# NeptuneHub/AudioMuse-AI

Measured on NVIDIA H100. Metric: tracks_per_sec_analysed_10s_48khz, higher is better.
Workload: dtype bf16

## Files before the change

### audiomuse-ai_b200/csrc/debug/block_debug.cu

```cuda
#include "../common.cuh"
#include "../depthwise.cuh"
#include "../fused_block.cuh"
#include "../gemm_wgmma.cuh"
#include "../model_spec.cuh"
#include "../../../include/audiomuse_b200_debug.h"

#include <vector>

namespace {

template <typename T>
int upload(am::DevBuf<T>& d, const void* h, size_t n) {
  AM_TRY(d.alloc(n));
  AM_CUDA(cudaMemcpy(d.p, h, n * sizeof(T), cudaMemcpyHostToDevice));
  return AM_OK;
}

template <typename T>
int download(void* h, const am::DevBuf<T>& d, size_t n) {
  AM_CUDA(cudaMemcpy(h, d.p, n * sizeof(T), cudaMemcpyDeviceToHost));
  return AM_OK;
}

}

extern "C" AM_API int am_debug_block(int path, int B, int H, int W, int cin_p, int cmid_p, int cout_p, int stride,
                                     int has_expand, int residual, const uint16_t* X, const uint16_t* W1,
                                     const float* b1, const float* wd, const float* bd, const uint16_t* W2,
                                     const float* b2, uint16_t* Y, uint16_t* E_out, uint16_t* D_out, int* info) {
  using namespace am;
  AM_CHECK(path >= 0 && path <= 2, "am_debug_block: path %d", path);
  AM_CHECK(B > 0 && H > 0 && W > 0 && (stride == 1 || stride == 2), "am_debug_block: bad shape");
  AM_CHECK(cin_p > 0 && cmid_p > 0 && cout_p > 0 && cin_p % 16 == 0 && cmid_p % 16 == 0 && cout_p % 16 == 0,
           "am_debug_block: channel counts must be positive multiples of 16");
  AM_CHECK(has_expand || cin_p == cmid_p, "am_debug_block: a block without expansion has cin_p == cmid_p");
  AM_CHECK(!residual || (stride == 1 && cin_p == cout_p), "am_debug_block: a residual needs stride 1, cin_p == cout_p");
  AM_CHECK(info, "am_debug_block: NULL info");

  fused::Plan pl;
  fused::BlockDesc d{};
  if (path != 1) {
    d.H = H;
    d.W = W;
    d.cin_p = cin_p;
    d.cmid_p = cmid_p;
    d.cout_p = cout_p;
    d.stride = stride;
    d.has_expand = has_expand ? 1 : 0;
    d.residual = residual ? 1 : 0;
    AM_CHECK(fused::plan(d, &pl), "am_debug_block: the fused kernel does not take this block");
    if (path == 2) {
      *info = pl.tile_h;
      return AM_OK;
    }
  }

  AM_CHECK(X && wd && bd && W2 && b2 && Y && (!has_expand || (W1 && b1)), "am_debug_block: NULL operand");
  AM_TRY(ensure_init());
  const int Ho = (H - 1) / stride + 1, Wo = (W - 1) / stride + 1;
  const size_t n_x = (size_t)B * H * W * cin_p, n_e = (size_t)B * H * W * cmid_p;
  const size_t n_d = (size_t)B * Ho * Wo * cmid_p, n_y = (size_t)B * Ho * Wo * cout_p;
  const std::vector<float> h_wd(wd, wd + (size_t)9 * cmid_p), h_bd(bd, bd + cmid_p);

  DevBuf<__nv_bfloat16> dX, dW1, dW2, dE, dD, dY;
  DevBuf<float> db1, dwd, dbd, db2, dparams;
  AM_TRY(upload(dX, X, n_x));
  AM_TRY(upload(dW2, W2, (size_t)cout_p * cmid_p));
  AM_TRY(upload(db2, b2, cout_p));
  if (has_expand) {
    AM_TRY(upload(dW1, W1, (size_t)cmid_p * cin_p));
    AM_TRY(upload(db1, b1, cmid_p));
  }
  AM_TRY(dY.alloc(n_y));
  AM_CUDA(cudaMemset(dY.p, 0xff, n_y * 2));

  if (path == 0) {
    const std::vector<float> h_b1 = has_expand ? std::vector<float>(b1, b1 + cmid_p) : std::vector<float>();
    const std::vector<float> packed = fused::pack_params(h_wd, h_bd, has_expand ? &h_b1 : nullptr, cmid_p);
    AM_TRY(upload(dparams, packed.data(), packed.size()));
    AM_TRY(fused::run(d, pl, dX.p, has_expand ? dW1.p : nullptr, dparams.p, dW2.p, db2.p, dY.p, B, nullptr));
    *info = pl.stages;
  } else {
    AM_TRY(upload(dwd, wd, (size_t)9 * cmid_p));
    AM_TRY(upload(dbd, bd, cmid_p));
    AM_TRY(dD.alloc(n_d));
    AM_CUDA(cudaMemset(dD.p, 0xff, n_d * 2));
    const __nv_bfloat16* dw_in = dX.p;
    if (has_expand) {
      AM_TRY(dE.alloc(n_e));
      AM_CUDA(cudaMemset(dE.p, 0xff, n_e * 2));
      gemm::Epilogue ep;
      ep.bias = db1.p;
      ep.act = kActRelu6;
      AM_TRY(gemm::gemm_bf16(dX.p, (int64_t)B * H * W, cin_p, dW1.p, cmid_p, cin_p, cin_p, dE.p, cmid_p, false, ep,
                             false, nullptr));
      dw_in = dE.p;
    }
    const bool fp16 = dw3x3_fp16_safe(h_wd, h_bd, cmid_p, has_expand != 0);
    AM_TRY(dw3x3(dw_in, B, H, W, cmid_p, stride, dwd.p, dbd.p, fp16, dD.p, nullptr, info));
    gemm::Epilogue ep;
    ep.bias = db2.p;
    if (residual) {
      ep.residual = dX.p;
      ep.ld_res = cout_p;
    }
    AM_TRY(gemm::gemm_bf16(dD.p, (int64_t)B * Ho * Wo, cmid_p, dW2.p, cout_p, cmid_p, cmid_p, dY.p, cout_p, false, ep,
                           false, nullptr));
  }
  AM_CUDA(cudaDeviceSynchronize());
  AM_TRY(download(Y, dY, n_y));
  if (path == 1 && E_out && has_expand) AM_TRY(download(E_out, dE, n_e));
  if (path == 1 && D_out) AM_TRY(download(D_out, dD, n_d));
  return AM_OK;
}
```

### audiomuse-ai_b200/csrc/fused_block.cu

```cuda
#include "fused_block.cuh"

#include <type_traits>

#include "gemm_wgmma.cuh"
#include "tma_pipeline.cuh"

namespace am {
namespace fused {

using namespace ptx;

constexpr int kTile = 8;
constexpr int kTallTile = 16;
constexpr int kChunk = 64;
constexpr int kMaxCout = 256;
constexpr int kMaxStages = 4;
constexpr size_t kSmemMax = 232448;
constexpr uint32_t kConsumerBar = 1;
constexpr int kParamRows = 9 + 1 + 1;
constexpr uint32_t kDwBytes = kParamRows * kChunk * 4;
using Ring = pipe::Ring<kMaxStages>;

__host__ __device__ constexpr int halo(int S) { return (kTile - 1) * S + 3; }
__host__ __device__ constexpr int halo_h(int S, int th) { return (th - 1) * S + 3; }
__host__ __device__ constexpr int halo_px(int S, int th) { return halo_h(S, th) * halo(S); }
__host__ __device__ constexpr int halo_rows(int S, int th) {
  return th == kTile ? (halo_px(S, th) + 63) / 64 * 64 : (halo_px(S, th) + 7) / 8 * 8;
}
__host__ __device__ constexpr int en0(int px) { return ((px + 7) / 8 + 1) / 2 * 8; }
__host__ __device__ constexpr int en1(int px) { return (px + 7) / 8 * 8 - en0(px); }

constexpr uint32_t round1k(uint32_t v) { return (v + 1023u) & ~1023u; }

__device__ __forceinline__ int e_off(int p, int g) { return p * 64 + ((g ^ (p & 7)) << 3); }

__device__ __forceinline__ uint32_t sw128(uint32_t row, uint32_t chunk) {
  return (row << 7) + (((chunk ^ row) & 7u) << 4);
}

struct Layout {
  uint32_t stage, w2, dw;
  uint32_t xs, a2, e, bars, extra;
  int hr;
  int th;
  int stages;
  size_t smem;
};

static Layout layout(int S, int th, bool has_expand, int cin_p, int cout_p, int stages) {
  const uint32_t hr = (uint32_t)halo_rows(S, th), hpx = (uint32_t)halo_px(S, th);
  const uint32_t kbx = has_expand ? (uint32_t)((cin_p + 63) / 64) : 0u;
  const uint32_t n2 = (uint32_t)((cout_p + 63) / 64 * 64);
  Layout l;
  l.w2 = has_expand ? kbx * kChunk * 128 : round1k(hpx * 128);
  l.dw = l.w2 + n2 * 128;
  l.stage = round1k(l.dw + kDwBytes);
  l.xs = 0;
  l.a2 = l.xs + kbx * hr * 128;
  l.e = l.a2 + (uint32_t)(th * kTile * 128);
  l.bars = l.e + (has_expand ? hpx * 128 : 0u);
  l.extra = l.bars + 2 * sizeof(uint64_t);
  l.hr = (int)hr;
  l.th = th;
  l.stages = stages;
  l.smem = Ring::smem_bytes(l.stage, stages, l.extra);
  return l;
}

struct Args {
  const __nv_bfloat16* X;
  const float* params;
  const float* b2;
  __nv_bfloat16* Y;
  int H, W, Ho, Wo, tiles_y, tiles_x, num_tiles;
  int cin_p, cmid_p, cout_p, residual;
  Layout l;
};

enum Phase { kRingWait, kHaloWait, kExpandMma, kExpandEpi, kDepthwise, kProjectMma, kBarrier, kEpilogue, kIssue, kNumPhases };
#ifdef AM_FUSED_PHASES
static const char* const kPhaseNames[kNumPhases] = {"ring_wait", "halo_wait", "expand_mma", "expand_epi", "depthwise",
                                                     "project_mma", "barrier", "epilogue", "issue"};
__device__ unsigned long long g_phase_cycles[3][kNumPhases];
__device__ __forceinline__ long long clock_now() {
  long long v;
  asm volatile("mov.u64 %0, %%clock64;" : "=l"(v));
  return v;
}
struct PhaseClock {
  uint32_t acc[kNumPhases];
  long long t;
  __device__ __forceinline__ PhaseClock() : acc{}, t(clock_now()) {}
  __device__ __forceinline__ void lap(Phase p) {
    const long long n = clock_now();
    acc[p] += (uint32_t)(n - t);
    t = n;
  }
  __device__ __forceinline__ void flush(int wg) {
    for (int p = 0; p < kNumPhases; ++p) atomicAdd(&g_phase_cycles[wg][p], (unsigned long long)acc[p]);
  }
};
#else
struct PhaseClock {
  __device__ __forceinline__ void lap(Phase) {}
  __device__ __forceinline__ void flush(int) {}
};
#endif

template <int S, bool kExpand>
__global__ void __launch_bounds__(pipe::kThreads, 1)
fused_block_kernel(const __grid_constant__ CUtensorMap map_x, const __grid_constant__ CUtensorMap map_w1,
                   const __grid_constant__ CUtensorMap map_w2, const Args a) {
  extern __shared__ __align__(1024) uint8_t smem_raw[];
  constexpr int HALO = halo(S);
  constexpr int PX8 = halo_px(S, kTile), PXT = halo_px(S, kTallTile);
  const bool tall = S == 1 && a.l.th == kTallTile;
  const int hpx = tall ? PXT : PX8, hr = a.l.hr;
  Ring ring(smem_raw, a.l.stage, a.l.stages, a.l.extra);
  uint8_t* own = ring.extra();
  uint8_t* xs = own + a.l.xs;
  uint8_t* a2 = own + a.l.a2;
  uint64_t* xs_full = reinterpret_cast<uint64_t*>(own + a.l.bars);
  uint64_t* xs_empty = xs_full + 1;

  const int per_img = a.tiles_y * a.tiles_x;
  const int kbx = (a.cin_p + 63) / 64;
  const int n2_blocks = (a.cout_p + 63) / 64;

  if (threadIdx.x == 0) {
    prefetch_tensormap(&map_x);
    if (kExpand) prefetch_tensormap(&map_w1);
    prefetch_tensormap(&map_w2);
    mbar_init(xs_full, 1);
    mbar_init(xs_empty, pipe::kConsumerThreads);
    ring.init();
  }
  __syncthreads();

  if (threadIdx.x < 128) {
    regs_producer();
    if (threadIdx.x < 32 && elect_one_sync()) {
      PhaseClock clk;
      uint32_t xs_phase = 0;
      for (int tile = blockIdx.x; tile < a.num_tiles; tile += gridDim.x) {
        const int b = tile / per_img, ty = (tile % per_img) / a.tiles_x, tx = tile % a.tiles_x;
        const int gy0 = ty * a.l.th * S - 1, gx0 = tx * kTile * S - 1;
        if (kExpand) {
          clk.lap(kIssue);
          mbar_wait(xs_empty, xs_phase ^ 1);
          clk.lap(kHaloWait);
          mbar_expect_tx(xs_full, (uint32_t)(kbx * hpx * 128));
          for (int kb = 0; kb < kbx; ++kb) tma_load_4d(xs + kb * hr * 128, &map_x, xs_full, kb * 64, gx0, gy0, b);
          xs_phase ^= 1;
        }
        for (int c0 = 0; c0 < a.cmid_p; c0 += kChunk) {
          const uint32_t tx_bytes = (kExpand ? (uint32_t)kbx * kChunk * 128 : (uint32_t)hpx * 128) +
                                    (uint32_t)n2_blocks * 64 * 128 + kDwBytes;
          clk.lap(kIssue);
          const Ring::Slot s = ring.acquire(tx_bytes);
          clk.lap(kRingWait);
          if (kExpand) {
            for (int kb = 0; kb < kbx; ++kb) tma_load_2d(s.smem + kb * kChunk * 128, &map_w1, s.bar, kb * 64, c0);
          } else {
            tma_load_4d(s.smem, &map_x, s.bar, c0, gx0, gy0, b);
          }
          tma_load_2d(s.smem + a.l.w2, &map_w2, s.bar, c0, 0);
          bulk_load(s.smem + a.l.dw, a.params + (int64_t)c0 * kParamRows, kDwBytes, s.bar);
        }
      }
      clk.lap(kIssue);
      clk.flush(0);
    }
    return;
  }
  regs_consumer();
  const int ct = threadIdx.x - 128;
  const int wg = __shfl_sync(0xffffffffu, ct >> 7, 0), wt = ct & 127;
  const int warp = wt >> 5, lane = wt & 31, quad = lane & 3;
  __nv_bfloat16* e_own = reinterpret_cast<__nv_bfloat16*>(own + a.l.e);
  const int nchunks = (a.cmid_p + kChunk - 1) / kChunk;
  const bool ahead = a.l.stages > 1;

  auto with_tile = [&](auto f) {
    if constexpr (S == 1) {
      if (tall) return f(std::integral_constant<int, kTallTile>{});
    }
    return f(std::integral_constant<int, kTile>{});
  };

  const int half = a.cout_p / 2;
  const int proj_n = tall ? a.cout_p : half;
  const int proj_col = tall ? 0 : wg * half;
  const int proj_row = tall ? 64 * wg : 0;

  constexpr int kAcc1 = en0(S == 1 ? PXT : PX8) / 2;
  float acc1[kAcc1];
  float acc2[kMaxCout / 4];
#pragma unroll
  for (int i = 0; i < kAcc1; ++i) acc1[i] = 0.f;
#pragma unroll
  for (int i = 0; i < kMaxCout / 4; ++i) acc2[i] = 0.f;

  auto expand_issue = [&](const uint8_t* stage) {
    const uint32_t w1 = smem_u32(stage);
    auto issue = [&](auto width, int p0) {
      const uint32_t px = smem_u32(xs) + (uint32_t)(p0 * 128);
      for (int kb = 0; kb < kbx; ++kb) {
        const uint64_t da = make_smem_desc(w1 + (uint32_t)(kb * kChunk * 128));
        const uint64_t db = make_smem_desc(px + (uint32_t)(kb * hr * 128));
        const int ksteps = min(4, (a.cin_p - kb * 64) / 16);
        for (int ks = 0; ks < ksteps; ++ks)
          wgmma_into<decltype(width)::value>(acc1, da + (uint64_t)(ks * 2), db + (uint64_t)(ks * 2),
                                             (kb | ks) ? 1u : 0u);
      }
    };
    wgmma_fence();
    with_tile([&](auto th) {
      constexpr int PX = halo_px(S, decltype(th)::value);
      if (wg == 0) issue(std::integral_constant<int, en0(PX)>{}, 0);
      else issue(std::integral_constant<int, en1(PX)>{}, en0(PX));
    });
    wgmma_commit();
  };
  auto inside_mask = [&](int gy0, int gx0) {
    return with_tile([&](auto th) {
      constexpr int EN0 = en0(halo_px(S, decltype(th)::value));
      int p0 = wg * EN0 + 2 * quad;
      asm volatile("" : "+r"(p0));
      uint64_t m = 0;
#pragma unroll
      for (int j = 0; j < EN0 / 8; ++j)
#pragma unroll
        for (int k = 0; k < 2; ++k) {
          const int p = p0 + 8 * j + k;
          const int gy = gy0 + p / HALO, gx = gx0 + p % HALO;
          if (gy >= 0 && gy < a.H && gx >= 0 && gx < a.W) m |= 1ull << (2 * j + k);
        }
      return m;
    });
  };
  auto expand_epilogue = [&](const uint8_t* stage, int nch, uint64_t inside) {
    reg_fence(acc1);
    const float* b1 = reinterpret_cast<const float*>(stage + a.l.dw) + 10 * kChunk;
    const int r = 16 * warp + (lane >> 2);
    const float bias[2] = {b1[r], b1[r + 8]};
    const uint32_t keep[2] = {r < nch ? ~0u : 0u, r + 8 < nch ? ~0u : 0u};
    auto pack = [&](int j, int h) {
      const uint32_t bits = (uint32_t)(inside >> (2 * j));
      const uint32_t mask = ((bits & 1u) * 0xffffu | (bits & 2u) * 0x7fff8000u) & keep[h];
      const __nv_bfloat162 v = __floats2bfloat162_rn(relu6f(acc1[4 * j + 2 * h] + bias[h]),
                                                     relu6f(acc1[4 * j + 2 * h + 1] + bias[h]));
      return *reinterpret_cast<const uint32_t*>(&v) & mask;
    };
    auto store = [&](auto wgc, auto th) {
      constexpr int HPX = halo_px(S, decltype(th)::value);
      constexpr int P0 = decltype(wgc)::value * en0(HPX);
      constexpr int NG = (decltype(wgc)::value ? en1(HPX) : en0(HPX)) / 8;
      constexpr int NFULL = (HPX - P0) / 8 < NG ? (HPX - P0) / 8 : NG;
      const int mi = lane >> 3;
      const uint32_t e_base = smem_u32(e_own);
#pragma unroll
      for (int j = 0; j + 1 < NFULL; j += 2) {
        const int p = P0 + 8 * (j + (mi >> 1)) + (lane & 7);
        stmatrix_x4_trans(e_base + 2 * e_off(p, 2 * warp + (mi & 1)), pack(j, 0), pack(j, 1), pack(j + 1, 0),
                          pack(j + 1, 1));
      }
      if (NFULL % 2) {
        const int p = P0 + 8 * (NFULL - 1) + (lane & 7);
        stmatrix_x2_trans(e_base + 2 * e_off(p, 2 * warp + (mi & 1)), pack(NFULL - 1, 0), pack(NFULL - 1, 1));
      }
#pragma unroll
      for (int j = NFULL; j < NG; ++j)
#pragma unroll
        for (int h = 0; h < 2; ++h) {
          const uint32_t v = pack(j, h);
#pragma unroll
          for (int k = 0; k < 2; ++k) {
            const int p = P0 + 8 * j + 2 * quad + k;
            if (p < HPX)
              reinterpret_cast<uint16_t*>(e_own)[e_off(p, 2 * warp + h) + (lane >> 2)] = (uint16_t)(v >> (16 * k));
          }
        }
    };
    with_tile([&](auto th) {
      if (wg == 0) store(std::integral_constant<int, 0>{}, th);
      else store(std::integral_constant<int, 1>{}, th);
    });
  };

  PhaseClock clk;
  uint32_t xs_phase = 0;
  for (int tile = blockIdx.x; tile < a.num_tiles; tile += gridDim.x) {
    const int b = tile / per_img, ty = (tile % per_img) / a.tiles_x, tx = tile % a.tiles_x;
    const int oy0 = ty * a.l.th, ox0 = tx * kTile;
    const int gy0 = oy0 * S - 1, gx0 = ox0 * S - 1;
    const uint64_t inside = kExpand ? inside_mask(gy0, gx0) : 0;
    if (kExpand) {
      mbar_wait(xs_full, xs_phase);
      xs_phase ^= 1;
      clk.lap(kHaloWait);
      const uint8_t* s0 = ring.wait_ptr();
      clk.lap(kRingWait);
      expand_issue(s0);
      wgmma_wait<0>();
      clk.lap(kExpandMma);
      expand_epilogue(s0, min(kChunk, a.cmid_p), inside);
      if (nchunks == 1) mbar_arrive(xs_empty);
      clk.lap(kExpandEpi);
    }

    for (int c = 0; c < nchunks; ++c) {
      const int c0 = c * kChunk, nch = min(kChunk, a.cmid_p - c0);
      const bool next = kExpand && c + 1 < nchunks;
      uint8_t* sp = ring.wait_ptr();
      clk.lap(kRingWait);
      const float* dwp = reinterpret_cast<const float*>(sp + a.l.dw);
      const __nv_bfloat16* e = kExpand ? e_own : reinterpret_cast<const __nv_bfloat16*>(sp);
      named_bar_sync(kConsumerBar, pipe::kConsumerThreads);
      clk.lap(kBarrier);
      const uint8_t* sn = nullptr;
      if (next && ahead) {
        sn = ring.wait_ahead_ptr();
        clk.lap(kRingWait);
        expand_issue(sn);
        clk.lap(kExpandMma);
      }

      with_tile([&](auto th) {
        constexpr int TH = decltype(th)::value, HH = halo_h(S, TH);
        const int ox = ct >> 5, cp = lane, g = cp >> 2;
        uint8_t* arow = a2 + sw128(ox, g) + 4 * (cp & 3);
        auto put = [&](int oy, uint32_t v) { *reinterpret_cast<uint32_t*>(arow + oy * kTile * 128) = v; };
        if (2 * cp < nch) {
          float2 w[9];
#pragma unroll
          for (int t = 0; t < 9; ++t) w[t] = *reinterpret_cast<const float2*>(dwp + t * kChunk + 2 * cp);
          const float2 bias = *reinterpret_cast<const float2*>(dwp + 9 * kChunk + 2 * cp);
          float2 acc[TH];
#pragma unroll
          for (int oy = 0; oy < TH; ++oy) acc[oy] = bias;
          auto out = [&](int oy) {
            const __nv_bfloat162 o = __floats2bfloat162_rn(relu6f(acc[oy].x), relu6f(acc[oy].y));
            return *reinterpret_cast<const uint32_t*>(&o);
          };
          const __nv_bfloat16* col[8];
#pragma unroll
          for (int k = 0; k < 8; ++k) col[k] = e + ox * S * 64 + ((g ^ ((ox * S + k) & 7)) << 3) + 2 * (cp & 3);
#pragma unroll
          for (int iy = 0; iy < HH; ++iy) {
            float2 v[3];
#pragma unroll
            for (int dx = 0; dx < 3; ++dx) {
              const int d = iy * HALO + dx;
              v[dx] = __bfloat1622float2(*reinterpret_cast<const __nv_bfloat162*>(col[d & 7] + d * 64));
            }
#pragma unroll
            for (int dy = 0; dy < 3; ++dy) {
              if (iy < dy || (iy - dy) % S != 0 || (iy - dy) / S >= TH) continue;
              const int oy = (iy - dy) / S;
#pragma unroll
              for (int dx = 0; dx < 3; ++dx) {
                acc[oy].x = fmaf(v[dx].x, w[dy * 3 + dx].x, acc[oy].x);
                acc[oy].y = fmaf(v[dx].y, w[dy * 3 + dx].y, acc[oy].y);
              }
            }
            if constexpr (TH != kTile) {
              if (iy >= 2) put(iy - 2, out(iy - 2));
            }
          }
          if constexpr (TH == kTile) {
#pragma unroll
            for (int oy = 0; oy < TH; ++oy) put(oy, out(oy));
          }
        } else {
#pragma unroll
          for (int oy = 0; oy < TH; ++oy) put(oy, 0u);
        }
      });
      fence_proxy_async();
      clk.lap(kDepthwise);
      named_bar_sync(kConsumerBar, pipe::kConsumerThreads);
      clk.lap(kBarrier);

      wgmma_fence();
      {
        const uint64_t da = make_smem_desc(smem_u32(a2) + (uint32_t)(proj_row * 128));
        const uint64_t db = make_smem_desc(smem_u32(sp) + a.l.w2 + (uint32_t)(proj_col * 128));
        auto project = [&](auto width) {
          for (int ks = 0; ks < nch / 16; ++ks)
            wgmma_into<decltype(width)::value>(acc2, da + (uint64_t)(ks * 2), db + (uint64_t)(ks * 2),
                                               (c0 | ks) ? 1u : 0u);
        };
        switch (proj_n) {
          case 8: project(std::integral_constant<int, 8>{}); break;
          case 16: project(std::integral_constant<int, 16>{}); break;
          case 24: project(std::integral_constant<int, 24>{}); break;
          case 32: project(std::integral_constant<int, 32>{}); break;
          case 40: project(std::integral_constant<int, 40>{}); break;
          case 48: project(std::integral_constant<int, 48>{}); break;
          case 56: project(std::integral_constant<int, 56>{}); break;
          case 64: project(std::integral_constant<int, 64>{}); break;
          case 72: project(std::integral_constant<int, 72>{}); break;
          case 80: project(std::integral_constant<int, 80>{}); break;
          case 88: project(std::integral_constant<int, 88>{}); break;
          case 96: project(std::integral_constant<int, 96>{}); break;
          case 104: project(std::integral_constant<int, 104>{}); break;
          case 112: project(std::integral_constant<int, 112>{}); break;
          case 120: project(std::integral_constant<int, 120>{}); break;
          case 128: project(std::integral_constant<int, 128>{}); break;
        }
      }
      wgmma_commit();
      clk.lap(kProjectMma);

      if (next && !ahead) {
        wgmma_wait<0>();
        ring.release();
        sn = ring.wait_ptr();
        clk.lap(kRingWait);
        expand_issue(sn);
      }
      wgmma_wait<0>();
      reg_fence(acc2);
      if (!next || ahead) ring.release();
      clk.lap(kProjectMma);
      if (next) {
        expand_epilogue(sn, min(kChunk, a.cmid_p - c0 - kChunk), inside);
        if (c + 2 == nchunks) mbar_arrive(xs_empty);
        clk.lap(kExpandEpi);
      }
    }

    {
      constexpr int J = kMaxCout / 16;
      bool in[2];
      int64_t pix[2];
#pragma unroll
      for (int h = 0; h < 2; ++h) {
        const int px = proj_row + warp * 16 + (lane >> 2) + 8 * h;
        const int oy = oy0 + (px >> 3), ox = ox0 + (px & 7);
        in[h] = oy < a.Ho && ox < a.Wo;
        pix[h] = ((int64_t)b * a.Ho + oy) * a.Wo + ox;
      }
      float2 bias[J];
      uint32_t res[2][J];
#pragma unroll
      for (int j = 0; j < J; ++j) {
        bias[j] = make_float2(0.f, 0.f);
        res[0][j] = res[1][j] = 0u;
        if (8 * j >= proj_n) continue;
        const int n = proj_col + 8 * j + 2 * quad;
        bias[j] = make_float2(__ldg(&a.b2[n]), __ldg(&a.b2[n + 1]));
#pragma unroll
        for (int h = 0; h < 2; ++h)
          if (a.residual && in[h]) res[h][j] = *reinterpret_cast<const uint32_t*>(a.X + pix[h] * a.cin_p + n);
      }
#pragma unroll
      for (int h = 0; h < 2; ++h) {
        if (!in[h]) continue;
#pragma unroll
        for (int j = 0; j < J; ++j) {
          if (8 * j >= proj_n) break;
          const int n = proj_col + 8 * j + 2 * quad;
          float f0 = acc2[4 * j + 2 * h] + bias[j].x;
          float f1 = acc2[4 * j + 2 * h + 1] + bias[j].y;
          if (a.residual) {
            f0 += __uint_as_float(res[h][j] << 16);
            f1 += __uint_as_float(res[h][j] & 0xffff0000u);
          }
          *reinterpret_cast<__nv_bfloat162*>(a.Y + pix[h] * a.cout_p + n) = __floats2bfloat162_rn(f0, f1);
        }
      }
    }
    clk.lap(kEpilogue);
  }
  if (wt == 0) clk.flush(1 + wg);
}

static bool fits(const BlockDesc& d) {
  const size_t hr = (size_t)halo_rows(d.stride, kTile);
  const size_t kbx = d.has_expand ? (size_t)((d.cin_p + 63) / 64) : 0;
  const size_t n2 = (size_t)((d.cout_p + 63) / 64 * 64);
  const size_t set = kbx * hr * 128 + kbx * kChunk * 128 + n2 * 128 + 64 * 128 + hr * 128;
  return set + 1024 <= kSmemMax;
}

bool plan(const BlockDesc& d, Plan* out) {
  if (d.stride != 1 && d.stride != 2) return false;
  if (d.cout_p > kMaxCout || d.cout_p % 16 || d.cmid_p % 16 || d.cin_p % 16) return false;
  if (!d.has_expand && d.cin_p != d.cmid_p) return false;
  if (d.residual && (d.stride != 1 || d.cin_p != d.cout_p)) return false;
  if (!fits(d)) return false;
  auto deepest = [&](int th) {
    Layout l = layout(d.stride, th, d.has_expand != 0, d.cin_p, d.cout_p, kMaxStages);
    for (int s = kMaxStages - 1; s >= 1 && l.smem > kSmemMax; --s)
      l = layout(d.stride, th, d.has_expand != 0, d.cin_p, d.cout_p, s);
    return l;
  };
  Layout l = deepest(kTile);
  if (d.stride == 1 && d.cout_p <= 128) {
    const Layout t = deepest(kTallTile);
    if (t.smem <= kSmemMax && t.stages == l.stages) l = t;
  }
  out->stages = l.stages;
  out->tile_h = l.th;
  out->smem_bytes = l.smem;
  return out->smem_bytes <= kSmemMax;
}

template <int S, bool kExpand>
static int launch(const CUtensorMap& mx, const CUtensorMap& m1, const CUtensorMap& m2, const Args& a, size_t smem,
                  cudaStream_t st) {
  AM_TRY((allow_dynamic_smem<fused_block_kernel<S, kExpand>>(kSmemMax)));
  const int grid = std::max(1, std::min(a.num_tiles, sm_count()));
#ifdef AM_FUSED_PHASES
  void* counters = nullptr;
  AM_CUDA(cudaGetSymbolAddress(&counters, g_phase_cycles));
  AM_CUDA(cudaMemsetAsync(counters, 0, sizeof(g_phase_cycles), st));
#endif
  AM_LAUNCH((fused_block_kernel<S, kExpand>), grid, pipe::kThreads, smem, st, mx, m1, m2, a);
#ifdef AM_FUSED_PHASES
  unsigned long long c[3][kNumPhases];
  AM_CUDA(cudaStreamSynchronize(st));
  AM_CUDA(cudaMemcpyFromSymbol(c, g_phase_cycles, sizeof(c)));
  std::fprintf(stderr, "fused_phases H=%d W=%d cin=%d cmid=%d cout=%d S=%d stages=%d grid=%d tiles=%d", a.H, a.W,
               a.cin_p, a.cmid_p, a.cout_p, S, a.l.stages, grid, a.num_tiles);
  for (int w = 0; w < 3; ++w)
    for (int p = 0; p < kNumPhases; ++p) std::fprintf(stderr, " wg%d.%s=%llu", w, kPhaseNames[p], c[w][p]);
  std::fprintf(stderr, "\n");
#endif
  return AM_OK;
}

std::vector<float> pack_params(const std::vector<float>& wd, const std::vector<float>& bd, const std::vector<float>* b1,
                               int c_p) {
  const int chunks = (c_p + kChunk - 1) / kChunk;
  std::vector<float> out((size_t)chunks * kParamRows * kChunk, 0.f);
  for (int c = 0; c < c_p; ++c) {
    float* q = &out[((size_t)(c / kChunk) * kParamRows) * kChunk + c % kChunk];
    for (int t = 0; t < 9; ++t) q[t * kChunk] = wd[(size_t)t * c_p + c];
    q[9 * kChunk] = bd[c];
    if (b1) q[10 * kChunk] = (*b1)[c];
  }
  return out;
}

int run(const BlockDesc& d, const Plan& p, const __nv_bfloat16* X, const __nv_bfloat16* W1, const float* params,
        const __nv_bfloat16* W2, const float* b2, __nv_bfloat16* Y, int B, cudaStream_t st) {
  AM_CHECK(X && params && W2 && b2 && Y && (!d.has_expand || W1), "fused block: NULL operand");
  auto aligned16 = [](const void* q) { return (reinterpret_cast<uintptr_t>(q) & 15) == 0; };
  AM_CHECK(aligned16(X) && aligned16(W2) && aligned16(params) && (!d.has_expand || aligned16(W1)),
           "fused block: operands must be 16-byte aligned (TMA)");
  Args a{};
  a.X = X;
  a.params = params;
  a.b2 = b2;
  a.Y = Y;
  a.H = d.H;
  a.W = d.W;
  a.Ho = (d.H - 1) / d.stride + 1;
  a.Wo = (d.W - 1) / d.stride + 1;
  AM_CHECK(p.tile_h == kTile || (p.tile_h == kTallTile && d.stride == 1 && d.cout_p <= 128),
           "fused block: plan does not match the block");
  a.tiles_y = (a.Ho + p.tile_h - 1) / p.tile_h;
  a.tiles_x = (a.Wo + kTile - 1) / kTile;
  const int64_t tiles = (int64_t)B * a.tiles_y * a.tiles_x;
  AM_CHECK(tiles < ((int64_t)1 << 31), "fused block: %lld tiles is too many for one launch", (long long)tiles);
  a.num_tiles = (int)tiles;
  a.cin_p = d.cin_p;
  a.cmid_p = d.cmid_p;
  a.cout_p = d.cout_p;
  a.residual = d.residual;
  const Layout l = layout(d.stride, p.tile_h, d.has_expand != 0, d.cin_p, d.cout_p, p.stages);
  AM_CHECK(l.smem == p.smem_bytes, "fused block: plan does not match the block");
  a.l = l;

  CUtensorMap mx, m1, m2;
  AM_TRY(gemm::encode_map_nhwc_bf16(&mx, X, B, d.H, d.W, d.cin_p, halo(d.stride), halo_h(d.stride, p.tile_h), true));
  AM_TRY(gemm::encode_map_bf16(&m2, W2, d.cmid_p, d.cout_p, d.cmid_p, (d.cout_p + 63) / 64 * 64));
  if (d.has_expand) AM_TRY(gemm::encode_map_bf16(&m1, W1, d.cin_p, d.cmid_p, d.cin_p, kChunk));
  else m1 = m2;
  if (d.stride == 1) return d.has_expand ? launch<1, true>(mx, m1, m2, a, l.smem, st) : launch<1, false>(mx, m1, m2, a, l.smem, st);
  return d.has_expand ? launch<2, true>(mx, m1, m2, a, l.smem, st) : launch<2, false>(mx, m1, m2, a, l.smem, st);
}

}
}
```

Baseline: 12090.

## Split depthwise rows across lanes for narrow chunks and stage output through smem

```diff
diff --git a/audiomuse-ai_b200/csrc/debug/block_debug.cu b/audiomuse-ai_b200/csrc/debug/block_debug.cu
--- a/audiomuse-ai_b200/csrc/debug/block_debug.cu
+++ b/audiomuse-ai_b200/csrc/debug/block_debug.cu
@@ -29,7 +29,7 @@
                                      const float* b1, const float* wd, const float* bd, const uint16_t* W2,
                                      const float* b2, uint16_t* Y, uint16_t* E_out, uint16_t* D_out, int* info) {
   using namespace am;
-  AM_CHECK(path >= 0 && path <= 2, "am_debug_block: path %d", path);
+  AM_CHECK(path >= 0 && path <= 3, "am_debug_block: path %d", path);
   AM_CHECK(B > 0 && H > 0 && W > 0 && (stride == 1 || stride == 2), "am_debug_block: bad shape");
   AM_CHECK(cin_p > 0 && cmid_p > 0 && cout_p > 0 && cin_p % 16 == 0 && cmid_p % 16 == 0 && cout_p % 16 == 0,
            "am_debug_block: channel counts must be positive multiples of 16");
@@ -49,8 +49,8 @@
     d.has_expand = has_expand ? 1 : 0;
     d.residual = residual ? 1 : 0;
     AM_CHECK(fused::plan(d, &pl), "am_debug_block: the fused kernel does not take this block");
-    if (path == 2) {
-      *info = pl.tile_h;
+    if (path >= 2) {
+      *info = path == 2 ? pl.tile_h : pl.stages;
       return AM_OK;
     }
   }
diff --git a/audiomuse-ai_b200/csrc/fused_block.cu b/audiomuse-ai_b200/csrc/fused_block.cu
--- a/audiomuse-ai_b200/csrc/fused_block.cu
+++ b/audiomuse-ai_b200/csrc/fused_block.cu
@@ -38,6 +38,8 @@
   return (row << 7) + (((chunk ^ row) & 7u) << 4);
 }
 
+__host__ __device__ constexpr uint32_t out_pitch(int cout_p) { return (uint32_t)cout_p * 2 + 16; }
+
 struct Layout {
   uint32_t stage, w2, dw;
   uint32_t xs, a2, e, bars, extra;
@@ -47,7 +49,7 @@
   size_t smem;
 };
 
-static Layout layout(int S, int th, bool has_expand, int cin_p, int cout_p, int stages) {
+static Layout layout(int S, int th, bool has_expand, bool residual, int cin_p, int cout_p, int stages) {
   const uint32_t hr = (uint32_t)halo_rows(S, th), hpx = (uint32_t)halo_px(S, th);
   const uint32_t kbx = has_expand ? (uint32_t)((cin_p + 63) / 64) : 0u;
   const uint32_t n2 = (uint32_t)((cout_p + 63) / 64 * 64);
@@ -58,7 +60,8 @@
   l.xs = 0;
   l.a2 = l.xs + kbx * hr * 128;
   l.e = l.a2 + (uint32_t)(th * kTile * 128);
-  l.bars = l.e + (has_expand ? hpx * 128 : 0u);
+  l.bars = std::max(l.e + (has_expand ? hpx * 128 : 0u),
+                    has_expand || residual ? 0u : l.a2 + (uint32_t)(th * kTile) * out_pitch(cout_p));
   l.extra = l.bars + 2 * sizeof(uint64_t);
   l.hr = (int)hr;
   l.th = th;
@@ -241,6 +244,7 @@
   };
   auto expand_epilogue = [&](const uint8_t* stage, int nch, uint64_t inside) {
     reg_fence(acc1);
+    if (16 * __shfl_sync(0xffffffffu, warp, 0) >= nch) return;
     const float* b1 = reinterpret_cast<const float*>(stage + a.l.dw) + 10 * kChunk;
     const int r = 16 * warp + (lane >> 2);
     const float bias[2] = {b1[r], b1[r + 8]};
@@ -326,26 +330,40 @@
         clk.lap(kExpandMma);
       }
 
-      with_tile([&](auto th) {
-        constexpr int TH = decltype(th)::value, HH = halo_h(S, TH);
-        const int ox = ct >> 5, cp = lane, g = cp >> 2;
-        uint8_t* arow = a2 + sw128(ox, g) + 4 * (cp & 3);
+      auto depthwise = [&](auto th, auto segs) {
+        constexpr int TH = decltype(th)::value, R = decltype(segs)::value, RT = TH / R, HH = halo_h(S, RT);
+        int ox, cp, oy0;
+        if constexpr (R == 1) {
+          ox = ct >> 5;
+          cp = lane;
+          oy0 = 0;
+        } else {
+          constexpr int NP = 32 / R, SETS = 8 / R;
+          const int w = ct >> 5, set = w % SETS, k = lane / NP;
+          cp = lane % NP;
+          oy0 = w / SETS * RT;
+          if constexpr (R == 4) ox = S == 1 ? set + 2 * k : ((0x6530 >> (4 * k)) & 7) ^ set;
+          else ox = S == 1 ? set + 4 * k : (k ? 4 + (set ^ 2) : set);
+        }
+        const int g = cp >> 2;
+        uint8_t* arow = a2 + sw128(ox, g) + 4 * (cp & 3) + oy0 * kTile * 128;
         auto put = [&](int oy, uint32_t v) { *reinterpret_cast<uint32_t*>(arow + oy * kTile * 128) = v; };
-        if (2 * cp < nch) {
+        if (R > 1 || 2 * cp < nch) {
           float2 w[9];
 #pragma unroll
           for (int t = 0; t < 9; ++t) w[t] = *reinterpret_cast<const float2*>(dwp + t * kChunk + 2 * cp);
           const float2 bias = *reinterpret_cast<const float2*>(dwp + 9 * kChunk + 2 * cp);
-          float2 acc[TH];
-#pragma unroll
-          for (int oy = 0; oy < TH; ++oy) acc[oy] = bias;
+          float2 acc[RT];
+#pragma unroll
+          for (int oy = 0; oy < RT; ++oy) acc[oy] = bias;
           auto out = [&](int oy) {
             const __nv_bfloat162 o = __floats2bfloat162_rn(relu6f(acc[oy].x), relu6f(acc[oy].y));
             return *reinterpret_cast<const uint32_t*>(&o);
           };
+          const int x0 = oy0 * S * HALO + ox * S;
           const __nv_bfloat16* col[8];
 #pragma unroll
-          for (int k = 0; k < 8; ++k) col[k] = e + ox * S * 64 + ((g ^ ((ox * S + k) & 7)) << 3) + 2 * (cp & 3);
+          for (int k = 0; k < 8; ++k) col[k] = e + x0 * 64 + ((g ^ ((x0 + k) & 7)) << 3) + 2 * (cp & 3);
 #pragma unroll
           for (int iy = 0; iy < HH; ++iy) {
             float2 v[3];
@@ -356,7 +374,7 @@
             }
 #pragma unroll
             for (int dy = 0; dy < 3; ++dy) {
-              if (iy < dy || (iy - dy) % S != 0 || (iy - dy) / S >= TH) continue;
+              if (iy < dy || (iy - dy) % S != 0 || (iy - dy) / S >= RT) continue;
               const int oy = (iy - dy) / S;
 #pragma unroll
               for (int dx = 0; dx < 3; ++dx) {
@@ -364,18 +382,23 @@
                 acc[oy].y = fmaf(v[dx].y, w[dy * 3 + dx].y, acc[oy].y);
               }
             }
-            if constexpr (TH != kTile) {
+            if constexpr (RT > kTile) {
               if (iy >= 2) put(iy - 2, out(iy - 2));
             }
           }
-          if constexpr (TH == kTile) {
-#pragma unroll
-            for (int oy = 0; oy < TH; ++oy) put(oy, out(oy));
+          if constexpr (RT <= kTile) {
+#pragma unroll
+            for (int oy = 0; oy < RT; ++oy) put(oy, out(oy));
           }
         } else {
 #pragma unroll
           for (int oy = 0; oy < TH; ++oy) put(oy, 0u);
         }
+      };
+      with_tile([&](auto th) {
+        if (nch == 16) depthwise(th, std::integral_constant<int, 4>{});
+        else if (nch == 32) depthwise(th, std::integral_constant<int, 2>{});
+        else depthwise(th, std::integral_constant<int, 1>{});
       });
       fence_proxy_async();
       clk.lap(kDepthwise);
@@ -431,7 +454,47 @@
       }
     }
 
-    {
+    const bool residual = S == 1 && a.residual;
+    if (!kExpand && !residual) {
+      constexpr int J = kMaxCout / 16;
+      const uint32_t pitch = out_pitch(a.cout_p);
+      auto for_pieces = [&](auto f) {
+        const int G = a.cout_p / 8, n = a.l.th * kTile * G;
+        const int dp = pipe::kConsumerThreads / G, dg = pipe::kConsumerThreads % G;
+        int p = ct / G, g = ct % G;
+        for (int i = ct; i < n; i += pipe::kConsumerThreads) {
+          const int oy = oy0 + (p >> 3), ox = ox0 + (p & 7);
+          if (oy < a.Ho && ox < a.Wo) f(a2 + p * pitch + 16 * g, ((int64_t)b * a.Ho + oy) * a.Wo + ox, 8 * g);
+          p += dp;
+          g += dg;
+          if (g >= G) {
+            g -= G;
+            ++p;
+          }
+        }
+      };
+      named_bar_sync(kConsumerBar, pipe::kConsumerThreads);
+      uint8_t* row = a2 + (proj_row + warp * 16 + (lane >> 2)) * pitch + 2 * (proj_col + 2 * quad);
+#pragma unroll
+      for (int j = 0; j < J; ++j) {
+        if (8 * j >= proj_n) break;
+        const int n = proj_col + 8 * j + 2 * quad;
+        const float2 bias = make_float2(__ldg(&a.b2[n]), __ldg(&a.b2[n + 1]));
+#pragma unroll
+        for (int h = 0; h < 2; ++h) {
+          uint32_t* s = reinterpret_cast<uint32_t*>(row + 8 * h * pitch + 16 * j);
+          float f0 = acc2[4 * j + 2 * h] + bias.x;
+          float f1 = acc2[4 * j + 2 * h + 1] + bias.y;
+          const __nv_bfloat162 v = __floats2bfloat162_rn(f0, f1);
+          *s = *reinterpret_cast<const uint32_t*>(&v);
+        }
+      }
+      named_bar_sync(kConsumerBar, pipe::kConsumerThreads);
+      for_pieces([&](const uint8_t* s, int64_t pix, int c) {
+        *reinterpret_cast<uint4*>(a.Y + pix * a.cout_p + c) = *reinterpret_cast<const uint4*>(s);
+      });
+    }
+    else {
       constexpr int J = kMaxCout / 16;
       bool in[2];
       int64_t pix[2];
@@ -453,7 +516,7 @@
         bias[j] = make_float2(__ldg(&a.b2[n]), __ldg(&a.b2[n + 1]));
 #pragma unroll
         for (int h = 0; h < 2; ++h)
-          if (a.residual && in[h]) res[h][j] = *reinterpret_cast<const uint32_t*>(a.X + pix[h] * a.cin_p + n);
+          if (residual && in[h]) res[h][j] = *reinterpret_cast<const uint32_t*>(a.X + pix[h] * a.cin_p + n);
       }
 #pragma unroll
       for (int h = 0; h < 2; ++h) {
@@ -464,7 +527,7 @@
           const int n = proj_col + 8 * j + 2 * quad;
           float f0 = acc2[4 * j + 2 * h] + bias[j].x;
           float f1 = acc2[4 * j + 2 * h + 1] + bias[j].y;
-          if (a.residual) {
+          if (residual) {
             f0 += __uint_as_float(res[h][j] << 16);
             f1 += __uint_as_float(res[h][j] & 0xffff0000u);
           }
@@ -492,9 +555,9 @@
   if (d.residual && (d.stride != 1 || d.cin_p != d.cout_p)) return false;
   if (!fits(d)) return false;
   auto deepest = [&](int th) {
-    Layout l = layout(d.stride, th, d.has_expand != 0, d.cin_p, d.cout_p, kMaxStages);
+    Layout l = layout(d.stride, th, d.has_expand != 0, d.residual != 0, d.cin_p, d.cout_p, kMaxStages);
     for (int s = kMaxStages - 1; s >= 1 && l.smem > kSmemMax; --s)
-      l = layout(d.stride, th, d.has_expand != 0, d.cin_p, d.cout_p, s);
+      l = layout(d.stride, th, d.has_expand != 0, d.residual != 0, d.cin_p, d.cout_p, s);
     return l;
   };
   Layout l = deepest(kTile);
@@ -549,8 +612,8 @@
         const __nv_bfloat16* W2, const float* b2, __nv_bfloat16* Y, int B, cudaStream_t st) {
   AM_CHECK(X && params && W2 && b2 && Y && (!d.has_expand || W1), "fused block: NULL operand");
   auto aligned16 = [](const void* q) { return (reinterpret_cast<uintptr_t>(q) & 15) == 0; };
-  AM_CHECK(aligned16(X) && aligned16(W2) && aligned16(params) && (!d.has_expand || aligned16(W1)),
-           "fused block: operands must be 16-byte aligned (TMA)");
+  AM_CHECK(aligned16(X) && aligned16(W2) && aligned16(params) && (!d.has_expand || aligned16(W1)) && aligned16(Y),
+           "fused block: operands must be 16-byte aligned (TMA, and 16-byte pieces of Y)");
   Args a{};
   a.X = X;
   a.params = params;
@@ -571,7 +634,7 @@
   a.cmid_p = d.cmid_p;
   a.cout_p = d.cout_p;
   a.residual = d.residual;
-  const Layout l = layout(d.stride, p.tile_h, d.has_expand != 0, d.cin_p, d.cout_p, p.stages);
+  const Layout l = layout(d.stride, p.tile_h, d.has_expand != 0, d.residual != 0, d.cin_p, d.cout_p, p.stages);
   AM_CHECK(l.smem == p.smem_bytes, "fused block: plan does not match the block");
   a.l = l;
 
```

Result: faster. 12310, median of 6 (+1.9%).
